# nihaomiao/CVPR23_LFDM

Measured on AMD Instinct MI355X. Metric: 40-frame 128x128 videos/sec (DDIM-100), higher is better.
Workload: dtype f32; 1 GPU; MUG 128x128, 40-frame DDIM-100 sample, batch=1 per GPU (BASELINE.json configs[1]); global_batch=1, frames=40, latent=32, image=128, sampler=DDIM-100 eta=1, cond_scale=1, parallelism=replicas x1 (videos sharded, no collective)

## Files before the change

cvpr23_lfdm_amd/csrc/attention.hip:

```cpp
#include <stdlib.h>
#include "attn_core.h"
#include "../../include/lfdm_hip.h"

namespace {

template <int LP>
__global__ __launch_bounds__(64) void attention_kernel(const float* __restrict__ qkv, float* __restrict__ out,
                                                       int frames, int hw, int mode, const float* __restrict__ bias,
                                                       const float* __restrict__ rot_cos,
                                                       const float* __restrict__ rot_sin) {
  constexpr int NT = LP / 16;

  const int lane = threadIdx.x & 63;
  const int l15 = lane & 15, lq = lane >> 4;
  const int L = mode == 0 ? frames : hw;
  const int64_t unit = blockIdx.x;
  const int64_t seq = unit / HEADS;
  const int head = (int)(unit - seq * HEADS);
  int64_t row0, tstride;
  if (mode == 0) {
    const int64_t b = seq / hw, pix = seq - b * hw;
    row0 = b * frames * hw + pix;
    tstride = hw;
  } else {
    row0 = seq * hw;
    tstride = 1;
  }
  const float* base = qkv + head * DH;

  float qf[NT][8], kf[NT][8];
#pragma unroll
  for (int ti = 0; ti < NT; ++ti) {
    const int t = ti * 16 + l15;
    float4 q0 = make_float4(0.f, 0.f, 0.f, 0.f), q1 = q0, k0 = q0, k1 = q0;
    if (t < L) {
      const float* src = base + (row0 + (int64_t)t * tstride) * QKV_LD + 8 * lq;
      q0 = *reinterpret_cast<const float4*>(src);
      q1 = *reinterpret_cast<const float4*>(src + 4);
      k0 = *reinterpret_cast<const float4*>(src + OUT_LD);
      k1 = *reinterpret_cast<const float4*>(src + OUT_LD + 4);
    }
    qf[ti][0] = q0.x * ATT_SCALE; qf[ti][1] = q0.y * ATT_SCALE; qf[ti][2] = q0.z * ATT_SCALE; qf[ti][3] = q0.w * ATT_SCALE;
    qf[ti][4] = q1.x * ATT_SCALE; qf[ti][5] = q1.y * ATT_SCALE; qf[ti][6] = q1.z * ATT_SCALE; qf[ti][7] = q1.w * ATT_SCALE;
    kf[ti][0] = k0.x; kf[ti][1] = k0.y; kf[ti][2] = k0.z; kf[ti][3] = k0.w;
    kf[ti][4] = k1.x; kf[ti][5] = k1.y; kf[ti][6] = k1.z; kf[ti][7] = k1.w;
  }
  float vf[2][4 * NT];
#pragma unroll
  for (int tj = 0; tj < NT; ++tj)
#pragma unroll
    for (int r = 0; r < 4; ++r) {
      const int t = 16 * tj + 4 * lq + r;
      vf[0][4 * tj + r] = vf[1][4 * tj + r] = 0.f;
      if (t < L) {
        const float* src = base + (row0 + (int64_t)t * tstride) * QKV_LD + 2 * OUT_LD;
        vf[0][4 * tj + r] = src[l15];
        vf[1][4 * tj + r] = src[16 + l15];
      }
    }
  if (rot_cos) {
#pragma unroll
    for (int ti = 0; ti < NT; ++ti) {
      const int t = ti * 16 + l15;
      if (t < L) {
#pragma unroll
        for (int pr = 0; pr < 4; ++pr) {
          const float c = rot_cos[t * 16 + 4 * lq + pr], sn = rot_sin[t * 16 + 4 * lq + pr];
          rot_pair(qf[ti][2 * pr], qf[ti][2 * pr + 1], c, sn);
          rot_pair(kf[ti][2 * pr], kf[ti][2 * pr + 1], c, sn);
        }
      }
    }
  }
  const bool bias_vec = bias && (L % 4 == 0) && ((((uintptr_t)bias) & 15) == 0);
  attend_store<NT, true>(qf, kf, vf, head, L, l15, lq, bias, bias_vec, out, row0, tstride);
}

__global__ __launch_bounds__(256) void linattn_context_kernel(const float* __restrict__ qkv, int hw,
                                                              float* __restrict__ ctx_out) {
  __shared__ float red[4][32];
  __shared__ float kmax[32];
  __shared__ float ek[64][33];
  __shared__ __attribute__((aligned(16))) float vv[64][36];
  const int tid = threadIdx.x;
  const int f = blockIdx.x >> 3, h = blockIdx.x & 7;
  const float* kbase = qkv + (int64_t)f * hw * QKV_LD + OUT_LD + h * DH;
  const float* vbase = kbase + OUT_LD;

  {
    const int c4 = tid & 7, part = tid >> 3;
    float4 m = make_float4(-3.0e38f, -3.0e38f, -3.0e38f, -3.0e38f);
    for (int n = part; n < hw; n += 128) {
      float4 v[4];
#pragma unroll
      for (int u = 0; u < 4; ++u) {
        const int nn = n + 32 * u;
        v[u] = nn < hw ? *reinterpret_cast<const float4*>(kbase + (int64_t)nn * QKV_LD + 4 * c4) : m;
      }
#pragma unroll
      for (int u = 0; u < 4; ++u) {
        m.x = fmaxf(m.x, v[u].x); m.y = fmaxf(m.y, v[u].y); m.z = fmaxf(m.z, v[u].z); m.w = fmaxf(m.w, v[u].w);
      }
    }
#pragma unroll
    for (int x = 8; x <= 32; x <<= 1) {
      m.x = fmaxf(m.x, __shfl_xor(m.x, x)); m.y = fmaxf(m.y, __shfl_xor(m.y, x));
      m.z = fmaxf(m.z, __shfl_xor(m.z, x)); m.w = fmaxf(m.w, __shfl_xor(m.w, x));
    }
    if ((tid & 63) < 8) {
      const int w = tid >> 6;
      red[w][4 * c4 + 0] = m.x; red[w][4 * c4 + 1] = m.y; red[w][4 * c4 + 2] = m.z; red[w][4 * c4 + 3] = m.w;
    }
    __syncthreads();
    if (tid < 32) kmax[tid] = fmaxf(fmaxf(red[0][tid], red[1][tid]), fmaxf(red[2][tid], red[3][tid]));
    __syncthreads();
  }

  const int d = tid >> 3, e0 = (tid & 7) * 4;
  float acc[4] = {0.f, 0.f, 0.f, 0.f};
  float ssum = 0.f;
  const int ln = tid >> 3, lc4 = tid & 7;
  float4 rk[2], rv[2];
  auto load_tile = [&](int n0) {
#pragma unroll
    for (int u = 0; u < 2; ++u) {
      const int n = n0 + ln + 32 * u;
      rk[u] = rv[u] = make_float4(0.f, 0.f, 0.f, 0.f);
      if (n < hw) {
// ... 53 lines not shown
  const int64_t row = (int64_t)f * hw + tok;
  const float* qp = qkv + row * QKV_LD + h * DH;
  float q[DH];
#pragma unroll
  for (int i = 0; i < DH / 4; ++i) {
    const float4 v = reinterpret_cast<const float4*>(qp)[i];
    q[4 * i] = v.x; q[4 * i + 1] = v.y; q[4 * i + 2] = v.z; q[4 * i + 3] = v.w;
  }
  float m = q[0];
#pragma unroll
  for (int i = 1; i < DH; ++i) m = fmaxf(m, q[i]);
  float sum = 0.f;
#pragma unroll
  for (int i = 0; i < DH; ++i) {
    q[i] = fast_exp(q[i] - m);
    sum += q[i];
  }
  const float scale = ATT_SCALE * fast_rcp(sum);
#pragma unroll
  for (int i = 0; i < DH; ++i) q[i] = q[i] * scale;
  float* op = out + row * OUT_LD + h * DH;
  const float* ch = cs + h * CS;
#pragma unroll
  for (int e4 = 0; e4 < DH / 4; ++e4) {
    float4 o = make_float4(0.f, 0.f, 0.f, 0.f);
#pragma unroll
    for (int dd = 0; dd < DH; ++dd) {
      const float4 c = *reinterpret_cast<const float4*>(ch + dd * DH + 4 * e4);
      o.x = fmaf(c.x, q[dd], o.x);
      o.y = fmaf(c.y, q[dd], o.y);
      o.z = fmaf(c.z, q[dd], o.z);
      o.w = fmaf(c.w, q[dd], o.w);
    }
    reinterpret_cast<float4*>(op)[e4] = o;
  }
}

}

extern "C" int lfdm_attention_cl_f32(const float* qkv, float* out, int batch, int frames, int hw,
                                     int mode, const float* bias, const float* rot_cos,
                                     const float* rot_sin, lfdm_stream_t stream_) {
  hipStream_t stream = (hipStream_t)stream_;
  const int L = mode == 0 ? frames : hw;
  if (!qkv || !out || batch <= 0 || frames <= 0 || hw <= 0 || (mode != 0 && mode != 1) ||
      L > 64 || ((rot_cos == nullptr) != (rot_sin == nullptr))) {
    lfdm_set_error("attention: unsupported shape (sequence length must be <= 64)");
    return LFDM_EINVAL;
  }
  const int64_t nseq = mode == 0 ? (int64_t)batch * hw : (int64_t)batch * frames;
  const int64_t units = nseq * HEADS;
  const dim3 grid((unsigned)units), block(64);
  lp_ladder(L, [&](auto lp) {
    LFDM_LAUNCH((attention_kernel<decltype(lp)::value>), grid, block, 0, stream, qkv, out, frames, hw, mode, bias, rot_cos, rot_sin);
  });
  return lfdm_check_launch("attention");
}

extern "C" size_t lfdm_linear_attention_ws_bytes(int n_frames) {
  return (size_t)n_frames * HEADS * DH * DH * sizeof(float);
}

extern "C" int lfdm_linear_attention_cl_f32(const float* qkv, float* out, int n_frames, int hw,
                                            void* ws, size_t ws_bytes, lfdm_stream_t stream_) {
  hipStream_t stream = (hipStream_t)stream_;
  if (!qkv || !out || n_frames <= 0 || hw <= 0) {
    lfdm_set_error("linear_attention: bad arguments");
    return LFDM_EINVAL;
  }
  if (!ws || ws_bytes < lfdm_linear_attention_ws_bytes(n_frames)) {
    lfdm_set_error("linear_attention: workspace too small");
    return LFDM_EWORKSPACE;
  }
  float* ctx = reinterpret_cast<float*>(ws);
  LFDM_LAUNCH(linattn_context_kernel, dim3(n_frames * HEADS), dim3(256), 0, stream, qkv, hw, ctx);
  LFDM_LAUNCH(linattn_output_kernel, dim3((hw + 31) / 32, n_frames), dim3(256), 0, stream, qkv,
              (const float*)ctx, hw, out);
  return lfdm_check_launch("linear_attention");
}
```

cvpr23_lfdm_amd/csrc/attention_fused.hip:

```cpp
#include <stdlib.h>

#include "attn_core.h"
#include "../../include/lfdm_hip.h"

namespace {

template <int LP, int C, bool ROT_RELOAD = false, bool WPACK = false>
__device__ __forceinline__ void tattn_heads(const float* __restrict__ x, int ldx, int head_begin, int heads_per_block,
                                            const float* __restrict__ wqkv, float* __restrict__ out, int frames, int hw, int64_t seq,
                                            const float* __restrict__ bias, const float* __restrict__ rot_cos,
                                            const float* __restrict__ rot_sin, float eps, float* o_lds) {
  constexpr int NT = LP / 16;
  constexpr int CQ = C / 4;

  const int lane = threadIdx.x & 63;
  const int l15 = lane & 15, lq = lane >> 4;
  const int L = frames;
  const int64_t b = seq / hw, pix = seq - b * hw;
  const int64_t row0 = b * frames * hw + pix;

  float xf[NT][CQ];
#pragma unroll
  for (int ti = 0; ti < NT; ++ti) {
    const int t = ti * 16 + l15;
    float s1 = 0.f, s2 = 0.f;
    if (t < L) {
      const float* src = x + (row0 + (int64_t)t * hw) * ldx + CQ * lq;
#pragma unroll
      for (int q = 0; q < CQ / 4; ++q) {
        const float4 v = *reinterpret_cast<const float4*>(src + 4 * q);
        xf[ti][4 * q] = v.x; xf[ti][4 * q + 1] = v.y; xf[ti][4 * q + 2] = v.z; xf[ti][4 * q + 3] = v.w;
        ln_accum(v, s1, s2);
      }
    } else {
#pragma unroll
      for (int s = 0; s < CQ; ++s) xf[ti][s] = 0.f;
    }
    float mean, rstd;
    ln_stats_slots4<false>(s1, s2, C, eps, mean, rstd);
    if (t < L) {
#pragma unroll
      for (int s = 0; s < CQ; ++s) xf[ti][s] = (xf[ti][s] - mean) * rstd;
    }
  }

  float rc[NT][4], rs[NT][4];
  if (rot_cos && !ROT_RELOAD) {
#pragma unroll
    for (int ti = 0; ti < NT; ++ti) {
      const int t = ti * 16 + l15;
      const int tt = t < L ? t : 0;
#pragma unroll
      for (int fi = 0; fi < 2; ++fi)
#pragma unroll
        for (int pr = 0; pr < 2; ++pr) {
          rc[ti][2 * fi + pr] = rot_cos[tt * 16 + 8 * fi + 2 * lq + pr];
          rs[ti][2 * fi + pr] = rot_sin[tt * 16 + 8 * fi + 2 * lq + pr];
        }
    }
  }
  const bool bias_vec = bias && (L % 4 == 0) && ((((uintptr_t)bias) & 15) == 0);

#pragma unroll 1
  for (int head = head_begin; head < head_begin + heads_per_block; ++head) {
    float qf[NT][8], kf[NT][8];
    {
      float wa[4][CQ];
#pragma unroll
      for (int g = 0; g < 4; ++g) {
        const float* wsrc = WPACK ? wqkv + ((int64_t)(((g >> 1) * HEADS + head) * 2 + (g & 1)) * (CQ / 4) * 64 + lane) * 4
                                  : wqkv + ((int64_t)((g >> 1) * OUT_LD + head * DH + 16 * (g & 1) + l15)) * C + CQ * lq;
#pragma unroll
        for (int q = 0; q < CQ / 4; ++q) {
          const float4 v = *reinterpret_cast<const float4*>(wsrc + (WPACK ? 256 * q : 4 * q));
          wa[g][4 * q] = v.x; wa[g][4 * q + 1] = v.y; wa[g][4 * q + 2] = v.z; wa[g][4 * q + 3] = v.w;
        }
      }
#pragma unroll
      for (int g = 0; g < 4; ++g) {
        f32x4 acc[NT];
#pragma unroll
        for (int ti = 0; ti < NT; ++ti) acc[ti] = (f32x4){0.f, 0.f, 0.f, 0.f};
#pragma unroll
        for (int s = 0; s < CQ; ++s)
#pragma unroll
          for (int ti = 0; ti < NT; ++ti) acc[ti] = mfma_16x16x4(wa[g][s], xf[ti][s], acc[ti]);
#pragma unroll
        for (int ti = 0; ti < NT; ++ti)
#pragma unroll
          for (int r = 0; r < 4; ++r) {
            if ((g >> 1) == 0) qf[ti][4 * (g & 1) + r] = acc[ti][r] * ATT_SCALE;
            else kf[ti][4 * (g & 1) + r] = acc[ti][r];
          }
      }
    }
    if (rot_cos) {
#pragma unroll
      for (int ti = 0; ti < NT; ++ti) {
#pragma unroll
        for (int fi = 0; fi < 2; ++fi)
#pragma unroll
          for (int pr = 0; pr < 2; ++pr) {
            float c, sn;
            if (ROT_RELOAD) {
              const int t = ti * 16 + l15, tt = t < L ? t : 0;
              c = rot_cos[tt * 16 + 8 * fi + 2 * lq + pr];
              sn = rot_sin[tt * 16 + 8 * fi + 2 * lq + pr];
            } else {
              c = rc[ti][2 * fi + pr];
              sn = rs[ti][2 * fi + pr];
            }
            rot_pair(qf[ti][4 * fi + 2 * pr], qf[ti][4 * fi + 2 * pr + 1], c, sn);
            rot_pair(kf[ti][4 * fi + 2 * pr], kf[ti][4 * fi + 2 * pr + 1], c, sn);
          }
      }
    }
    float vf[2][4 * NT];
    {
      float wb[2][CQ];
#pragma unroll
      for (int half = 0; half < 2; ++half) {
        const float* wsrc = WPACK ? wqkv + ((int64_t)((2 * HEADS + head) * 2 + half) * (CQ / 4) * 64 + lane) * 4
                                  : wqkv + ((int64_t)(2 * OUT_LD + head * DH + 16 * half + l15)) * C + CQ * lq;
#pragma unroll
        for (int q = 0; q < CQ / 4; ++q) {
          const float4 v = *reinterpret_cast<const float4*>(wsrc + (WPACK ? 256 * q : 4 * q));
          wb[half][4 * q] = v.x; wb[half][4 * q + 1] = v.y; wb[half][4 * q + 2] = v.z; wb[half][4 * q + 3] = v.w;
        }
      }
#pragma unroll
      for (int half = 0; half < 2; ++half) {
        f32x4 acc[NT];
#pragma unroll
        for (int ti = 0; ti < NT; ++ti) acc[ti] = (f32x4){0.f, 0.f, 0.f, 0.f};
#pragma unroll
        for (int s = 0; s < CQ; ++s)
#pragma unroll
          for (int ti = 0; ti < NT; ++ti) acc[ti] = mfma_16x16x4(xf[ti][s], wb[half][s], acc[ti]);
#pragma unroll
        for (int ti = 0; ti < NT; ++ti)
#pragma unroll
          for (int r = 0; r < 4; ++r) vf[half][4 * ti + r] = acc[ti][r];
      }
    }

    attend_store<NT, false>(qf, kf, vf, head, L, l15, lq, bias, bias_vec, out, row0, hw, o_lds);
  }
}

template <int LP, int C>
__global__ __launch_bounds__(64, 2) void temporal_attn_fused_kernel(const float* __restrict__ x, int ldx, int heads_per_block,
                                                                 const float* __restrict__ wqkv,
                                                                 float* __restrict__ out, int frames, int hw,
                                                                 const float* __restrict__ bias,
                                                                 const float* __restrict__ rot_cos,
                                                                 const float* __restrict__ rot_sin, float eps) {
  tattn_heads<LP, C>(x, ldx, blockIdx.y * heads_per_block, heads_per_block, wqkv, out, frames, hw, blockIdx.x, bias, rot_cos, rot_sin, eps, nullptr);
}

template <int LP, int LROWS, int NW>
__global__ __launch_bounds__(64 * NW, 2) void temporal_attn_fused_out_kernel(const float* __restrict__ x, int ldx,
                                                                          const float* __restrict__ wqkv, const float* __restrict__ wout,
                                                                          float* __restrict__ out, int ldo, int frames, int hw,
                                                                          const float* __restrict__ bias, const float* __restrict__ rot_cos,
                                                                          const float* __restrict__ rot_sin, float eps) {
  constexpr int C = 64, NT = LP / 16, CT = C / 16;
  __shared__ __attribute__((aligned(16))) float o_lds[LROWS * OUT_LD];
  const int wave = lfdm_uniform((int)(threadIdx.x >> 6));
  const int lane = threadIdx.x & 63, l15 = lane & 15, lq = lane >> 4;
  const int L = frames;
  const int64_t seq = blockIdx.x;
  tattn_heads<LP, C, (NW < 8), true>(x, ldx, wave * (HEADS / NW), HEADS / NW, wqkv, nullptr, frames, hw, seq, bias, rot_cos, rot_sin, eps, o_lds);
  __syncthreads();
  const int64_t b = seq / hw, pix = seq - b * hw;
  const int64_t row0 = b * frames * hw + pix;
  for (int tile = wave; tile < NT * CT; tile += NW) {
    const int ti = tile / CT, ct = tile - ti * CT;
    const int t = ti * 16 + l15;
    const int tr = t < L ? t : L - 1;
    const float* arow = o_lds + tr * OUT_LD;
    const float* brow = wout + ((int64_t)ct * (OUT_LD / 16) * 64 + lane) * 4;
    f32x4 acc = {0.f, 0.f, 0.f, 0.f}, acc1 = acc;
    float xr[4];
#pragma unroll
    for (int r = 0; r < 4; ++r) {
      const int tok = ti * 16 + 4 * lq + r;
      xr[r] = x[(row0 + (int64_t)(tok < L ? tok : L - 1) * hw) * ldx + ct * 16 + l15];
    }
#pragma unroll 4
    for (int S = 0; S < OUT_LD / 16; S += 2) {
      const float4 a = *reinterpret_cast<const float4*>(arow + (((4 * S + lq) ^ (tr & 15)) << 2));
      const float4 a1 = *reinterpret_cast<const float4*>(arow + (((4 * S + 4 + lq) ^ (tr & 15)) << 2));
      const float4 w = *reinterpret_cast<const float4*>(brow + 256 * S);
      const float4 w1 = *reinterpret_cast<const float4*>(brow + 256 * S + 256);
      acc = mfma_16x16x4(a.x, w.x, acc);
      acc1 = mfma_16x16x4(a1.x, w1.x, acc1);
      acc = mfma_16x16x4(a.y, w.y, acc);
      acc1 = mfma_16x16x4(a1.y, w1.y, acc1);
      acc = mfma_16x16x4(a.z, w.z, acc);
      acc1 = mfma_16x16x4(a1.z, w1.z, acc1);
      acc = mfma_16x16x4(a.w, w.w, acc);
      acc1 = mfma_16x16x4(a1.w, w1.w, acc1);
    }
#pragma unroll
    for (int r = 0; r < 4; ++r) acc[r] += acc1[r];
#pragma unroll
    for (int r = 0; r < 4; ++r) {
      const int tok = ti * 16 + 4 * lq + r;
      if (tok < L) {
        const int64_t row = row0 + (int64_t)tok * hw;
        out[row * ldo + ct * 16 + l15] = acc[r] + xr[r];
      }
    }
  }
}

template <int LP>
__global__ __launch_bounds__(64, 1) void temporal_attn_fused_wide_kernel(const float* __restrict__ x, int ldx, int channels,
                                                                      int heads_per_block, const float* __restrict__ wqkv,
                                                                      float* __restrict__ out, int frames, int hw,
                                                                      const float* __restrict__ bias,
                                                                      const float* __restrict__ rot_cos,
                                                                      const float* __restrict__ rot_sin, float eps) {
  constexpr int NT = LP / 16;
  const int lane = threadIdx.x & 63;
  const int l15 = lane & 15, lq = lane >> 4;
  const int L = frames;
  const int64_t seq = blockIdx.x;
  const int64_t b = seq / hw, pix = seq - b * hw;
  const int64_t row0 = b * frames * hw + pix;
  const int ncb = channels / 64;

  float mean[NT], rstd[NT];
#pragma unroll
  for (int ti = 0; ti < NT; ++ti) {
    const int t = ti * 16 + l15;
    float s1 = 0.f, s2 = 0.f;
    if (t < L) {
      const float* src = x + (row0 + (int64_t)t * hw) * ldx + 16 * lq;
      for (int cb = 0; cb < ncb; ++cb)
#pragma unroll
        for (int q = 0; q < 4; ++q) ln_accum(*reinterpret_cast<const float4*>(src + 64 * cb + 4 * q), s1, s2);
    }
    ln_stats_slots4<true>(s1, s2, channels, eps, mean[ti], rstd[ti]);
  }
  const bool bias_vec = bias && (L % 4 == 0) && ((((uintptr_t)bias) & 15) == 0);

  const int head_begin = blockIdx.y * heads_per_block;
#pragma unroll 1
  for (int head = head_begin; head < head_begin + heads_per_block; ++head) {
    f32x4 aq[2][NT], ak[2][NT], av[2][NT];
#pragma unroll
    for (int g = 0; g < 2; ++g)
#pragma unroll
      for (int ti = 0; ti < NT; ++ti) aq[g][ti] = ak[g][ti] = av[g][ti] = (f32x4){0.f, 0.f, 0.f, 0.f};
#pragma unroll 1
    for (int cb = 0; cb < ncb; ++cb) {
      float w[6][16];
#pragma unroll
      for (int g = 0; g < 6; ++g) {
        const float* wsrc = wqkv + ((int64_t)((g >> 1) * OUT_LD + head * DH + 16 * (g & 1) + l15)) * channels + 64 * cb + 16 * lq;
#pragma unroll
        for (int q = 0; q < 4; ++q) {
          const float4 v = *reinterpret_cast<const float4*>(wsrc + 4 * q);
          w[g][4 * q] = v.x; w[g][4 * q + 1] = v.y; w[g][4 * q + 2] = v.z; w[g][4 * q + 3] = v.w;
        }
      }
#pragma unroll
      for (int ti = 0; ti < NT; ++ti) {
        const int t = ti * 16 + l15;
        float xf[16];
        if (t < L) {
          const float* src = x + (row0 + (int64_t)t * hw) * ldx + 64 * cb + 16 * lq;
#pragma unroll
          for (int q = 0; q < 4; ++q) {
            const float4 v = *reinterpret_cast<const float4*>(src + 4 * q);
            xf[4 * q] = (v.x - mean[ti]) * rstd[ti]; xf[4 * q + 1] = (v.y - mean[ti]) * rstd[ti];
            xf[4 * q + 2] = (v.z - mean[ti]) * rstd[ti]; xf[4 * q + 3] = (v.w - mean[ti]) * rstd[ti];
          }
        } else {
#pragma unroll
          for (int s2 = 0; s2 < 16; ++s2) xf[s2] = 0.f;
        }
#pragma unroll
        for (int s2 = 0; s2 < 16; ++s2) {
          aq[0][ti] = mfma_16x16x4(w[0][s2], xf[s2], aq[0][ti]);
          aq[1][ti] = mfma_16x16x4(w[1][s2], xf[s2], aq[1][ti]);
          ak[0][ti] = mfma_16x16x4(w[2][s2], xf[s2], ak[0][ti]);
          ak[1][ti] = mfma_16x16x4(w[3][s2], xf[s2], ak[1][ti]);
          av[0][ti] = mfma_16x16x4(xf[s2], w[4][s2], av[0][ti]);
          av[1][ti] = mfma_16x16x4(xf[s2], w[5][s2], av[1][ti]);
        }
      }
    }
    float qf[NT][8], kf[NT][8], vf[2][4 * NT];
#pragma unroll
    for (int ti = 0; ti < NT; ++ti)
#pragma unroll
      for (int fi = 0; fi < 2; ++fi)
#pragma unroll
        for (int r = 0; r < 4; ++r) {
          qf[ti][4 * fi + r] = aq[fi][ti][r] * ATT_SCALE;
          kf[ti][4 * fi + r] = ak[fi][ti][r];
          vf[fi][4 * ti + r] = av[fi][ti][r];
        }
    if (rot_cos) {
#pragma unroll
      for (int ti = 0; ti < NT; ++ti) {
        const int t = ti * 16 + l15;
        const int tt = t < L ? t : 0;
#pragma unroll
        for (int fi = 0; fi < 2; ++fi)
#pragma unroll
          for (int pr = 0; pr < 2; ++pr) {
            const float c = rot_cos[tt * 16 + 8 * fi + 2 * lq + pr], sn = rot_sin[tt * 16 + 8 * fi + 2 * lq + pr];
            rot_pair(qf[ti][4 * fi + 2 * pr], qf[ti][4 * fi + 2 * pr + 1], c, sn);
            rot_pair(kf[ti][4 * fi + 2 * pr], kf[ti][4 * fi + 2 * pr + 1], c, sn);
          }
      }
    }
    attend_store<NT, false>(qf, kf, vf, head, L, l15, lq, bias, bias_vec, out, row0, hw);
  }
}

int launch_fused_wide(const float* x, int ldx, int channels, const float* wqkv, float* out, int batch, int frames, int hw,
                      const float* bias, const float* rot_cos, const float* rot_sin, float eps, hipStream_t stream) {
  const int64_t nseq = (int64_t)batch * hw;
  int hpb = 8;
  while (hpb > 1 && nseq * (HEADS / hpb) < 2048) hpb >>= 1;
  const dim3 grid((unsigned)nseq, (unsigned)(HEADS / hpb)), block(64);
  lp_ladder(frames, [&](auto lp) {
    LFDM_LAUNCH((temporal_attn_fused_wide_kernel<decltype(lp)::value>), grid, block, 0, stream, x, ldx, channels, hpb, wqkv, out, frames, hw, bias, rot_cos, rot_sin, eps);
  });
  return lfdm_check_launch("temporal_attention_fused_wide");
}

template <int C>
int launch_fused(const float* x, int ldx, const float* wqkv, float* out, int batch, int frames, int hw, const float* bias,
                 const float* rot_cos, const float* rot_sin, float eps, hipStream_t stream) {
  const int64_t nseq = (int64_t)batch * hw;
  int hpb = 8;
  while (hpb > 1 && nseq * (HEADS / hpb) < 2048) hpb >>= 1;
  if (const char* e = lfdm_knob("LFDM_TATTN_HPB")) {
    const int v = atoi(e);
    if (v == 1 || v == 2 || v == 4 || v == 8) hpb = v;
  }
  const dim3 grid((unsigned)nseq, (unsigned)(HEADS / hpb)), block(64);
  lp_ladder(frames, [&](auto lp) {
    LFDM_LAUNCH((temporal_attn_fused_kernel<decltype(lp)::value, C>), grid, block, 0, stream, x, ldx, hpb, wqkv, out, frames, hw, bias, rot_cos, rot_sin, eps);
  });
  return lfdm_check_launch("temporal_attention_fused");
}

template <int LP, int LROWS>
int launch_fused_out_lp(const float* x, int ldx, const float* wqkv, const float* wout, float* out, int ldo, int batch, int frames, int hw,
                        const float* bias, const float* rot_cos, const float* rot_sin, float eps, hipStream_t stream) {
  const int64_t nseq = (int64_t)batch * hw;
  int nw = 2;
  while (nw < 8 && nseq * nw < 2048) nw <<= 1;
  if (const char* e = getenv("LFDM_TATTN_OUT_NW")) {
    const int v = atoi(e);
    if (v == 1 || v == 2 || v == 4 || v == 8) nw = v;
  }
  const dim3 grid((unsigned)nseq);
  lfdm_ladder<1, 2, 4, 8>(nw, [&](auto nwc) {
    constexpr int NW = decltype(nwc)::value;
    LFDM_LAUNCH((temporal_attn_fused_out_kernel<LP, LROWS, NW>), grid, dim3(64 * NW), 0, stream, x, ldx, wqkv, wout, out, ldo, frames, hw, bias, rot_cos, rot_sin, eps);
  });
  return lfdm_check_launch("temporal_attention_fused_out");
}

}

extern "C" int lfdm_temporal_attention_fused_out_cl_f32(const float* x, int ldx, int channels, const float* wqkv, const float* wout,
                                                        float* out, int ldo, int batch, int frames, int hw, const float* bias,
                                                        const float* rot_cos, const float* rot_sin, float ln_eps, lfdm_stream_t stream_) {
  hipStream_t stream = (hipStream_t)stream_;
  if (!x || !wqkv || !wout || !out || batch <= 0 || frames <= 0 || frames > 64 || hw <= 0 || channels != 64 || ldx < 64 || ldx % 4 != 0 ||
      ldo < 64 || (((uintptr_t)x | (uintptr_t)wqkv | (uintptr_t)wout) & 15) || ((rot_cos == nullptr) != (rot_sin == nullptr)) || out == x) {
    lfdm_set_error("temporal_attention_fused_out: needs C == 64, frames <= 64, 16-byte aligned rows, out != x");
    return LFDM_EINVAL;
  }
  return lp_ladder(frames, [&](auto lp) {
    constexpr int LP = decltype(lp)::value;
    if (LP == 48 && frames <= 40)
      return launch_fused_out_lp<48, 40>(x, ldx, wqkv, wout, out, ldo, batch, frames, hw, bias, rot_cos, rot_sin, ln_eps, stream);
    return launch_fused_out_lp<LP, LP>(x, ldx, wqkv, wout, out, ldo, batch, frames, hw, bias, rot_cos, rot_sin, ln_eps, stream);
  });
}

extern "C" int lfdm_temporal_attention_fused_cl_f32(const float* x, int ldx, int channels, const float* wqkv, float* out,
                                                    int batch, int frames, int hw, const float* bias,
                                                    const float* rot_cos, const float* rot_sin, float ln_eps,
                                                    lfdm_stream_t stream_) {
  hipStream_t stream = (hipStream_t)stream_;
  if (!x || !wqkv || !out || batch <= 0 || frames <= 0 || frames > 64 || hw <= 0 || ldx < channels || ldx % 4 != 0 ||
      (((uintptr_t)x | (uintptr_t)wqkv) & 15) || ((rot_cos == nullptr) != (rot_sin == nullptr)) ||
      channels < 64 || channels % 64 != 0) {
    lfdm_set_error("temporal_attention_fused: needs C % 64 == 0, frames <= 64, 16-byte aligned rows");
    return LFDM_EINVAL;
  }
  if (channels == 64) return launch_fused<64>(x, ldx, wqkv, out, batch, frames, hw, bias, rot_cos, rot_sin, ln_eps, stream);
  return launch_fused_wide(x, ldx, channels, wqkv, out, batch, frames, hw, bias, rot_cos, rot_sin, ln_eps, stream);
}
```

cvpr23_lfdm_amd/csrc/attn_core.h:

```cpp
#pragma once
#include "lfdm_device.h"

constexpr int HEADS = 8;
constexpr int DH = 32;
constexpr int QKV_LD = 3 * HEADS * DH;
constexpr int OUT_LD = HEADS * DH;
constexpr float ATT_SCALE = 0.17677669529663687f;

__device__ __forceinline__ void seq_rows(int64_t seq, int mode, int frames, int hw, int64_t& row0, int64_t& tstride) {
  if (mode == 0) {
    const int64_t b = seq / hw, pix = seq - b * hw;
    row0 = b * frames * hw + pix;
    tstride = hw;
  } else {
    row0 = seq * hw;
    tstride = 1;
  }
}

__device__ __forceinline__ void rot_pair(float& x, float& y, float c, float sn) {
  const float x0 = x, y0 = y;
  x = x0 * c - y0 * sn;
  y = y0 * c + x0 * sn;
}

template <int NT, bool FAST_RCP>
__device__ __forceinline__ float softmax_tile(f32x4 (&st)[NT], int head, int L, int qt, int lq, const float* __restrict__ bias, bool bias_vec) {
  float m = -3.0e38f;
#pragma unroll
  for (int tj = 0; tj < NT; ++tj) {
    float bv[4] = {0.f, 0.f, 0.f, 0.f};
    const int key0 = tj * 16 + lq * 4;
    if (bias && qt < L && key0 < L) {
      const float* bp = bias + ((int64_t)head * L + qt) * L + key0;
      if (bias_vec) {
        const float4 b4 = *reinterpret_cast<const float4*>(bp);
        bv[0] = b4.x; bv[1] = b4.y; bv[2] = b4.z; bv[3] = b4.w;
      } else {
#pragma unroll
        for (int r = 0; r < 4; ++r) bv[r] = (key0 + r < L) ? bp[r] : 0.f;
      }
    }
#pragma unroll
    for (int r = 0; r < 4; ++r) {
      const float v = (key0 + r >= L) ? -3.0e38f : st[tj][r] + bv[r];
      st[tj][r] = v;
      m = fmaxf(m, v);
    }
  }
  m = fmaxf(m, __shfl_xor(m, 16));
  m = fmaxf(m, __shfl_xor(m, 32));
  float sum = 0.f;
#pragma unroll
  for (int tj = 0; tj < NT; ++tj)
#pragma unroll
    for (int r = 0; r < 4; ++r) {
      const float e = (tj * 16 + lq * 4 + r) < L ? fast_exp(st[tj][r] - m) : 0.f;
      st[tj][r] = e;
      sum += e;
    }
  sum += __shfl_xor(sum, 16);
  sum += __shfl_xor(sum, 32);
  return FAST_RCP ? fast_rcp(sum) : 1.0f / sum;
}

template <int NT, bool FAST_RCP>
__device__ __forceinline__ void attend_store(const float (&qf)[NT][8], const float (&kf)[NT][8], const float (&vf)[2][4 * NT],
                                             int head, int L, int l15, int lq, const float* __restrict__ bias, bool bias_vec,
                                             float* __restrict__ out, int64_t row0, int64_t tstride, float* o_lds = nullptr) {
  f32x4 st[NT][NT];
#pragma unroll
  for (int ti = 0; ti < NT; ++ti)
#pragma unroll
    for (int tj = 0; tj < NT; ++tj) {
      f32x4 acc = {0.f, 0.f, 0.f, 0.f};
#pragma unroll
      for (int s = 0; s < 8; ++s) acc = mfma_16x16x4(kf[tj][s], qf[ti][s], acc);
      st[ti][tj] = acc;
    }
#pragma unroll
  for (int ti = 0; ti < NT; ++ti) {
    const float inv = softmax_tile<NT, FAST_RCP>(st[ti], head, L, ti * 16 + l15, lq, bias, bias_vec);
#pragma unroll
    for (int tj = 0; tj < NT; ++tj)
#pragma unroll
      for (int r = 0; r < 4; ++r) st[ti][tj][r] = st[ti][tj][r] * inv;
  }

#pragma unroll
  for (int ti = 0; ti < NT; ++ti) {
    f32x4 o[2];
    o[0] = (f32x4){0.f, 0.f, 0.f, 0.f};
    o[1] = o[0];
#pragma unroll
    for (int tj = 0; tj < NT; ++tj)
#pragma unroll
      for (int r = 0; r < 4; ++r) {
        o[0] = mfma_16x16x4(st[ti][tj][r], vf[0][4 * tj + r], o[0]);
        o[1] = mfma_16x16x4(st[ti][tj][r], vf[1][4 * tj + r], o[1]);
      }
#pragma unroll
    for (int r = 0; r < 4; ++r) {
      const int t = ti * 16 + lq * 4 + r;
      if (t < L) {
        if (o_lds) {
#pragma unroll
          for (int half = 0; half < 2; ++half) {
            const int c = head * DH + 16 * half + l15;
            o_lds[t * OUT_LD + ((((c >> 2) ^ (t & 15)) << 2) | (c & 3))] = o[half][r];
          }
        } else {
          float* dst = out + (row0 + t * tstride) * OUT_LD + head * DH;
          dst[l15] = o[0][r];
          dst[16 + l15] = o[1][r];
        }
      }
    }
  }
}

__device__ __forceinline__ void ln_accum(const float4& v, float& s1, float& s2) {
  s1 += (v.x + v.y) + (v.z + v.w);
  s2 += (v.x * v.x + v.y * v.y) + (v.z * v.z + v.w * v.w);
}
template <bool DIVIDE>
__device__ __forceinline__ void ln_stats_slots4(float s1, float s2, int channels, float eps, float& mean, float& rstd) {
  s1 += __shfl_xor(s1, 16); s2 += __shfl_xor(s2, 16);
  s1 += __shfl_xor(s1, 32); s2 += __shfl_xor(s2, 32);
  mean = DIVIDE ? s1 / (float)channels : s1 * (1.0f / (float)channels);
  float var = (DIVIDE ? s2 / (float)channels : s2 * (1.0f / (float)channels)) - mean * mean;
  if (var < 0.f) var = 0.f;
  rstd = 1.0f / sqrtf(var + eps);
}

template <class F>
inline auto lp_ladder(int L, F&& f) { return lfdm_ladder<16, 32, 48, 64>(L, f); }
```

cvpr23_lfdm_amd/csrc/lfdm_device.h:

```cpp
#pragma once
#include <stddef.h>
#include <stdint.h>
#include <type_traits>

#if defined(LFDM_EMU_BUILD)
#include "hip_emu.h"
typedef emu_f32x16 f32x16;
typedef emu_f32x4 f32x4;
#define LFDM_LAUNCH(kern, grid, block, smem, stream, ...) \
  emu::launch(grid, block, smem, [=]() { kern(__VA_ARGS__); })
static inline f32x16 mfma_32x32x2(float a, float b, f32x16 c) { return emu_mfma_32x32x2(a, b, c); }
static inline f32x4 mfma_16x16x4(float a, float b, f32x4 c) { return emu_mfma_16x16x4(a, b, c); }
static inline f32x4 mfma_4x4x1(float a, float b, f32x4 c) { return emu_mfma_4x4x1(a, b, c); }
struct lfdm_bf16x8 { uint16_t h[8]; };
static inline uint16_t lfdm_f32_to_bf16(float f) {
  uint32_t u;
  memcpy(&u, &f, 4);
  if ((u & 0x7fffffffu) > 0x7f800000u) return (uint16_t)((u >> 16) | 0x40u);
  u += 0x7fffu + ((u >> 16) & 1u);
  return (uint16_t)(u >> 16);
}
static inline float lfdm_bf16_to_f32(uint16_t h) {
  const uint32_t u = (uint32_t)h << 16;
  float f;
// ... 152 lines not shown
__device__ __forceinline__ void lfdm_gload_f4(f32x4& dst, const float* p) {
  asm volatile("global_load_dwordx4 %0, %1, off offset:%2" : "=v"(dst) : "v"(p), "n"(OFF) : "memory");
}
template <int N> __device__ __forceinline__ void lfdm_vmwait() { asm volatile("s_waitcnt vmcnt(%0)" ::"n"(N) : "memory"); }
template <int N> __device__ __forceinline__ void lfdm_vmwait(f32x4& a) { asm volatile("s_waitcnt vmcnt(%1)" : "+v"(a) : "n"(N) : "memory"); }
template <int N> __device__ __forceinline__ void lfdm_vmwait(f32x4& a, f32x4& b) {
  asm volatile("s_waitcnt vmcnt(%2)" : "+v"(a), "+v"(b) : "n"(N) : "memory");
}
template <int N> __device__ __forceinline__ void lfdm_vmwait(f32x4& a, f32x4& b, f32x4& c, f32x4& d) {
  asm volatile("s_waitcnt vmcnt(%4)" : "+v"(a), "+v"(b), "+v"(c), "+v"(d) : "n"(N) : "memory");
}
__device__ __forceinline__ void lfdm_tie(f32x4& a) { asm volatile("" : "+v"(a)::"memory"); }
__device__ __forceinline__ int lfdm_uniform(int v) { return __builtin_amdgcn_readfirstlane(v); }
#endif

#if defined(LFDM_EMU_BUILD)
#define LFDM_DRAIN_STORES() ((void)0)
#define LFDM_FENCE_RELEASE_AGENT() ((void)0)
#define LFDM_FENCE_ACQUIRE_AGENT() ((void)0)
static inline unsigned lfdm_ticket_take(unsigned* c) { return __atomic_fetch_add(c, 1u, __ATOMIC_SEQ_CST); }
static inline void lfdm_ticket_reset(unsigned* c) { __atomic_store_n(c, 0u, __ATOMIC_SEQ_CST); }
#else
#define LFDM_DRAIN_STORES() asm volatile("s_waitcnt vmcnt(0)" ::: "memory")
#define LFDM_FENCE_RELEASE_AGENT() __builtin_amdgcn_fence(__ATOMIC_RELEASE, "agent")
#define LFDM_FENCE_ACQUIRE_AGENT() __builtin_amdgcn_fence(__ATOMIC_ACQUIRE, "agent")
__device__ __forceinline__ unsigned lfdm_ticket_take(unsigned* c) {
  return __hip_atomic_fetch_add(c, 1u, __ATOMIC_RELAXED, __HIP_MEMORY_SCOPE_AGENT);
}
__device__ __forceinline__ void lfdm_ticket_reset(unsigned* c) {
  __hip_atomic_store(c, 0u, __ATOMIC_RELAXED, __HIP_MEMORY_SCOPE_AGENT);
}
#endif

#if defined(__HIP_DEVICE_COMPILE__) && !defined(__gfx950__) && !defined(LFDM_EMU_BUILD)
#error "fence-free hand-off (lfdm_agent_store_u64 / lfdm_agent_load_u64 / lfdm_ticket_take) validated on gfx950 only: re-validate, or use LFDM_FENCE_RELEASE_AGENT / LFDM_FENCE_ACQUIRE_AGENT, before building for another target"
#endif
#if defined(LFDM_EMU_BUILD)
static inline void lfdm_agent_store_u64(unsigned long long* p, unsigned long long v) { __atomic_store_n(p, v, __ATOMIC_SEQ_CST); }
static inline unsigned long long lfdm_agent_load_u64(const unsigned long long* p) { return __atomic_load_n(p, __ATOMIC_SEQ_CST); }
static inline unsigned lfdm_agent_load_u32(const unsigned* p) { return __atomic_load_n(p, __ATOMIC_SEQ_CST); }
static inline void lfdm_sleep() {}
#else
__device__ __forceinline__ void lfdm_agent_store_u64(unsigned long long* p, unsigned long long v) {
  __hip_atomic_store(p, v, __ATOMIC_RELAXED, __HIP_MEMORY_SCOPE_AGENT);
}
__device__ __forceinline__ unsigned long long lfdm_agent_load_u64(const unsigned long long* p) {
  return __hip_atomic_load(p, __ATOMIC_RELAXED, __HIP_MEMORY_SCOPE_AGENT);
}
__device__ __forceinline__ unsigned lfdm_agent_load_u32(const unsigned* p) { return __hip_atomic_load(p, __ATOMIC_RELAXED, __HIP_MEMORY_SCOPE_AGENT); }
__device__ __forceinline__ void lfdm_sleep() { __builtin_amdgcn_s_sleep(2); }
#endif

#if defined(LFDM_EMU_BUILD)
static inline void lfdm_wave_lds_sync() { emu::wave_sync(); }
#else
__device__ __forceinline__ void lfdm_wave_lds_sync() {
  __builtin_amdgcn_fence(__ATOMIC_RELEASE, "wavefront");
  __builtin_amdgcn_wave_barrier();
  __builtin_amdgcn_fence(__ATOMIC_ACQUIRE, "wavefront");
}
#endif

__device__ __forceinline__ float wave_sum(float v) {
#pragma unroll
  for (int m = 32; m >= 1; m >>= 1) v += __shfl_xor(v, m);
  return v;
}
__device__ __forceinline__ float wave_max(float v) {
#pragma unroll
  for (int m = 32; m >= 1; m >>= 1) v = fmaxf(v, __shfl_xor(v, m));
  return v;
}
#if defined(LFDM_EMU_BUILD)
static inline float fast_exp(float x) { return expf(x); }
static inline float fast_rcp(float x) { return 1.0f / x; }
#else
__device__ __forceinline__ float fast_exp(float x) { return __expf(x); }
__device__ __forceinline__ float fast_rcp(float x) { return __builtin_amdgcn_rcpf(x); }
#endif
__device__ __forceinline__ float sigmoidf_(float x) { return 1.0f / (1.0f + expf(-x)); }
__device__ __forceinline__ float siluf_(float x) { return x / (1.0f + expf(-x)); }

#if defined(LFDM_EMU_BUILD)
static inline float silu_fast_(float x) { return x / (1.0f + expf(-x)); }
#else
__device__ __forceinline__ float silu_fast_(float x) { return x * __builtin_amdgcn_rcpf(1.0f + __expf(-x)); }
#endif

#if defined(LFDM_TUNING_KNOBS) || defined(LFDM_EMU_BUILD)
static inline const char* lfdm_knob(const char* name) { return getenv(name); }
#else
static inline const char* lfdm_knob(const char*) { return nullptr; }
#endif

__device__ __forceinline__ float apply_act(float v, int act) {
  if (act == 1) return v > 0.f ? v : 0.f;
  if (act == 2) return sigmoidf_(v);
  if (act == 3) return siluf_(v);
  return v;
}

extern "C" void lfdm_set_error(const char* msg);
int lfdm_check_launch(const char* what);
```

Baseline: 4.125 videos/s.

## Software-pipeline attention score MFMA with softmax VALU per query tile

```diff
diff --git a/cvpr23_lfdm_amd/csrc/attention.hip b/cvpr23_lfdm_amd/csrc/attention.hip
--- a/cvpr23_lfdm_amd/csrc/attention.hip
+++ b/cvpr23_lfdm_amd/csrc/attention.hip
@@ -4,7 +4,7 @@
 
 namespace {
 
-template <int LP>
+template <int LP, bool PIPE>
 __global__ __launch_bounds__(64) void attention_kernel(const float* __restrict__ qkv, float* __restrict__ out,
                                                        int frames, int hw, int mode, const float* __restrict__ bias,
                                                        const float* __restrict__ rot_cos,
@@ -73,7 +73,7 @@
     }
   }
   const bool bias_vec = bias && (L % 4 == 0) && ((((uintptr_t)bias) & 15) == 0);
-  attend_store<NT, true>(qf, kf, vf, head, L, l15, lq, bias, bias_vec, out, row0, tstride);
+  attend_store<NT, true, PIPE>(qf, kf, vf, head, L, l15, lq, bias, bias_vec, out, row0, tstride);
 }
 
 __global__ __launch_bounds__(256) void linattn_context_kernel(const float* __restrict__ qkv, int hw,
@@ -233,7 +233,12 @@
   const int64_t units = nseq * HEADS;
   const dim3 grid((unsigned)units), block(64);
   lp_ladder(L, [&](auto lp) {
-    LFDM_LAUNCH((attention_kernel<decltype(lp)::value>), grid, block, 0, stream, qkv, out, frames, hw, mode, bias, rot_cos, rot_sin);
+    constexpr int LP = decltype(lp)::value;
+    constexpr bool CAN_PIPE = LP != 32;
+    if (CAN_PIPE && bias_by_quads(bias, L))
+      LFDM_LAUNCH((attention_kernel<LP, CAN_PIPE>), grid, block, 0, stream, qkv, out, frames, hw, mode, bias, rot_cos, rot_sin);
+    else
+      LFDM_LAUNCH((attention_kernel<LP, false>), grid, block, 0, stream, qkv, out, frames, hw, mode, bias, rot_cos, rot_sin);
   });
   return lfdm_check_launch("attention");
 }
diff --git a/cvpr23_lfdm_amd/csrc/attention_fused.hip b/cvpr23_lfdm_amd/csrc/attention_fused.hip
--- a/cvpr23_lfdm_amd/csrc/attention_fused.hip
+++ b/cvpr23_lfdm_amd/csrc/attention_fused.hip
@@ -5,11 +5,34 @@
 
 namespace {
 
-template <int LP, int C, bool ROT_RELOAD = false, bool WPACK = false>
+#ifdef LFDM_TATTN_STAMP
+struct CycleProbe {
+  long long t, acc[8];
+  __device__ __forceinline__ void start() {
+    for (int i = 0; i < 8; ++i) acc[i] = 0;
+    t = clock64();
+  }
+  __device__ __forceinline__ void lap(int i) {
+    LFDM_SCHED_FENCE();
+    const long long now = clock64();
+    acc[i] += now - t;
+    t = now;
+    LFDM_SCHED_FENCE();
+  }
+};
+long long* tattn_stamps = nullptr;
+#define TATTN_STAMP_PARAM , long long* stamps
+#define TATTN_STAMP_ARG , tattn_stamps
+#else
+#define TATTN_STAMP_PARAM
+#define TATTN_STAMP_ARG
+#endif
+
+template <int LP, int C, bool ROT_RELOAD = false, bool WPACK = false, bool PIPE = false, bool TO_LDS = false, class PROBE = NoProbe>
 __device__ __forceinline__ void tattn_heads(const float* __restrict__ x, int ldx, int head_begin, int heads_per_block,
                                             const float* __restrict__ wqkv, float* __restrict__ out, int frames, int hw, int64_t seq,
                                             const float* __restrict__ bias, const float* __restrict__ rot_cos,
-                                            const float* __restrict__ rot_sin, float eps, float* o_lds) {
+                                            const float* __restrict__ rot_sin, float eps, PROBE&& probe = NoProbe{}) {
   constexpr int NT = LP / 16;
   constexpr int CQ = C / 4;
 
@@ -60,6 +83,7 @@
     }
   }
   const bool bias_vec = bias && (L % 4 == 0) && ((((uintptr_t)bias) & 15) == 0);
+  probe.lap(4);
 
 #pragma unroll 1
   for (int head = head_begin; head < head_begin + heads_per_block; ++head) {
@@ -144,34 +168,42 @@
       }
     }
 
-    attend_store<NT, false>(qf, kf, vf, head, L, l15, lq, bias, bias_vec, out, row0, hw, o_lds);
-  }
-}
-
-template <int LP, int C>
+    probe.lap(0);
+    attend_store<NT, false, PIPE, TO_LDS>(qf, kf, vf, head, L, l15, lq, bias, bias_vec, out, row0, hw, probe);
+  }
+}
+
+template <int LP, int C, bool PIPE>
 __global__ __launch_bounds__(64, 2) void temporal_attn_fused_kernel(const float* __restrict__ x, int ldx, int heads_per_block,
                                                                  const float* __restrict__ wqkv,
                                                                  float* __restrict__ out, int frames, int hw,
                                                                  const float* __restrict__ bias,
                                                                  const float* __restrict__ rot_cos,
                                                                  const float* __restrict__ rot_sin, float eps) {
-  tattn_heads<LP, C>(x, ldx, blockIdx.y * heads_per_block, heads_per_block, wqkv, out, frames, hw, blockIdx.x, bias, rot_cos, rot_sin, eps, nullptr);
-}
-
-template <int LP, int LROWS, int NW>
+  tattn_heads<LP, C, false, false, PIPE>(x, ldx, blockIdx.y * heads_per_block, heads_per_block, wqkv, out, frames, hw, blockIdx.x, bias, rot_cos, rot_sin, eps);
+}
+
+template <int LP, int LROWS, int NW, bool PIPE>
 __global__ __launch_bounds__(64 * NW, 2) void temporal_attn_fused_out_kernel(const float* __restrict__ x, int ldx,
                                                                           const float* __restrict__ wqkv, const float* __restrict__ wout,
                                                                           float* __restrict__ out, int ldo, int frames, int hw,
                                                                           const float* __restrict__ bias, const float* __restrict__ rot_cos,
-                                                                          const float* __restrict__ rot_sin, float eps) {
+                                                                          const float* __restrict__ rot_sin, float eps TATTN_STAMP_PARAM) {
   constexpr int C = 64, NT = LP / 16, CT = C / 16;
   __shared__ __attribute__((aligned(16))) float o_lds[LROWS * OUT_LD];
   const int wave = lfdm_uniform((int)(threadIdx.x >> 6));
   const int lane = threadIdx.x & 63, l15 = lane & 15, lq = lane >> 4;
   const int L = frames;
   const int64_t seq = blockIdx.x;
-  tattn_heads<LP, C, (NW < 8), true>(x, ldx, wave * (HEADS / NW), HEADS / NW, wqkv, nullptr, frames, hw, seq, bias, rot_cos, rot_sin, eps, o_lds);
+#ifdef LFDM_TATTN_STAMP
+  CycleProbe probe;
+  probe.start();
+#else
+  NoProbe probe;
+#endif
+  tattn_heads<LP, C, (NW < 8), true, PIPE, true>(x, ldx, wave * (HEADS / NW), HEADS / NW, wqkv, o_lds, frames, hw, seq, bias, rot_cos, rot_sin, eps, probe);
   __syncthreads();
+  probe.lap(5);
   const int64_t b = seq / hw, pix = seq - b * hw;
   const int64_t row0 = b * frames * hw + pix;
   for (int tile = wave; tile < NT * CT; tile += NW) {
@@ -213,9 +245,14 @@
       }
     }
   }
-}
-
-template <int LP>
+#ifdef LFDM_TATTN_STAMP
+  probe.lap(6);
+  if (stamps && lane == 0 && blockIdx.x < 256)
+    for (int i = 0; i < 8; ++i) stamps[((int64_t)blockIdx.x * 8 + wave) * 8 + i] = probe.acc[i];
+#endif
+}
+
+template <int LP, bool PIPE>
 __global__ __launch_bounds__(64, 1) void temporal_attn_fused_wide_kernel(const float* __restrict__ x, int ldx, int channels,
                                                                       int heads_per_block, const float* __restrict__ wqkv,
                                                                       float* __restrict__ out, int frames, int hw,
@@ -319,7 +356,7 @@
           }
       }
     }
-    attend_store<NT, false>(qf, kf, vf, head, L, l15, lq, bias, bias_vec, out, row0, hw);
+    attend_store<NT, false, PIPE>(qf, kf, vf, head, L, l15, lq, bias, bias_vec, out, row0, hw);
   }
 }
 
@@ -330,7 +367,11 @@
   while (hpb > 1 && nseq * (HEADS / hpb) < 2048) hpb >>= 1;
   const dim3 grid((unsigned)nseq, (unsigned)(HEADS / hpb)), block(64);
   lp_ladder(frames, [&](auto lp) {
-    LFDM_LAUNCH((temporal_attn_fused_wide_kernel<decltype(lp)::value>), grid, block, 0, stream, x, ldx, channels, hpb, wqkv, out, frames, hw, bias, rot_cos, rot_sin, eps);
+    constexpr int LP = decltype(lp)::value;
+    if (bias_by_quads(bias, frames))
+      LFDM_LAUNCH((temporal_attn_fused_wide_kernel<LP, true>), grid, block, 0, stream, x, ldx, channels, hpb, wqkv, out, frames, hw, bias, rot_cos, rot_sin, eps);
+    else
+      LFDM_LAUNCH((temporal_attn_fused_wide_kernel<LP, false>), grid, block, 0, stream, x, ldx, channels, hpb, wqkv, out, frames, hw, bias, rot_cos, rot_sin, eps);
   });
   return lfdm_check_launch("temporal_attention_fused_wide");
 }
@@ -347,7 +388,12 @@
   }
   const dim3 grid((unsigned)nseq, (unsigned)(HEADS / hpb)), block(64);
   lp_ladder(frames, [&](auto lp) {
-    LFDM_LAUNCH((temporal_attn_fused_kernel<decltype(lp)::value, C>), grid, block, 0, stream, x, ldx, hpb, wqkv, out, frames, hw, bias, rot_cos, rot_sin, eps);
+    constexpr int LP = decltype(lp)::value;
+    constexpr bool CAN_PIPE = LP <= 32;
+    if (CAN_PIPE && bias_by_quads(bias, frames))
+      LFDM_LAUNCH((temporal_attn_fused_kernel<LP, C, CAN_PIPE>), grid, block, 0, stream, x, ldx, hpb, wqkv, out, frames, hw, bias, rot_cos, rot_sin, eps);
+    else
+      LFDM_LAUNCH((temporal_attn_fused_kernel<LP, C, false>), grid, block, 0, stream, x, ldx, hpb, wqkv, out, frames, hw, bias, rot_cos, rot_sin, eps);
   });
   return lfdm_check_launch("temporal_attention_fused");
 }
@@ -365,12 +411,24 @@
   const dim3 grid((unsigned)nseq);
   lfdm_ladder<1, 2, 4, 8>(nw, [&](auto nwc) {
     constexpr int NW = decltype(nwc)::value;
-    LFDM_LAUNCH((temporal_attn_fused_out_kernel<LP, LROWS, NW>), grid, dim3(64 * NW), 0, stream, x, ldx, wqkv, wout, out, ldo, frames, hw, bias, rot_cos, rot_sin, eps);
+#if defined(LFDM_TATTN_STAMP) && LFDM_TATTN_STAMP == 2
+    constexpr bool CAN_PIPE = false;
+#else
+    constexpr bool CAN_PIPE = !(LP == 64 && NW == 4);
+#endif
+    if (CAN_PIPE && bias_by_quads(bias, frames))
+      LFDM_LAUNCH((temporal_attn_fused_out_kernel<LP, LROWS, NW, CAN_PIPE>), grid, dim3(64 * NW), 0, stream, x, ldx, wqkv, wout, out, ldo, frames, hw, bias, rot_cos, rot_sin, eps TATTN_STAMP_ARG);
+    else
+      LFDM_LAUNCH((temporal_attn_fused_out_kernel<LP, LROWS, NW, false>), grid, dim3(64 * NW), 0, stream, x, ldx, wqkv, wout, out, ldo, frames, hw, bias, rot_cos, rot_sin, eps TATTN_STAMP_ARG);
   });
   return lfdm_check_launch("temporal_attention_fused_out");
 }
 
 }
+
+#ifdef LFDM_TATTN_STAMP
+extern "C" void lfdm_tattn_stamp_buffer(void* p) { tattn_stamps = (long long*)p; }
+#endif
 
 extern "C" int lfdm_temporal_attention_fused_out_cl_f32(const float* x, int ldx, int channels, const float* wqkv, const float* wout,
                                                         float* out, int ldo, int batch, int frames, int hw, const float* bias,
diff --git a/cvpr23_lfdm_amd/csrc/attn_core.h b/cvpr23_lfdm_amd/csrc/attn_core.h
--- a/cvpr23_lfdm_amd/csrc/attn_core.h
+++ b/cvpr23_lfdm_amd/csrc/attn_core.h
@@ -24,14 +24,18 @@
   y = y0 * c + x0 * sn;
 }
 
-template <int NT, bool FAST_RCP>
-__device__ __forceinline__ float softmax_tile(f32x4 (&st)[NT], int head, int L, int qt, int lq, const float* __restrict__ bias, bool bias_vec) {
-  float m = -3.0e38f;
+template <int NT, bool GUARDED>
+__device__ __forceinline__ void bias_quads(f32x4 (&bq)[NT], int head, int L, int qt, int lq, const float* __restrict__ bias, bool bias_vec,
+                                           bool clamp_q = true) {
 #pragma unroll
   for (int tj = 0; tj < NT; ++tj) {
-    float bv[4] = {0.f, 0.f, 0.f, 0.f};
+    f32x4 bv = {0.f, 0.f, 0.f, 0.f};
     const int key0 = tj * 16 + lq * 4;
-    if (bias && qt < L && key0 < L) {
+    if (!GUARDED) {
+      const float* brow = bias + ((int64_t)head * L + (clamp_q && qt > L - 1 ? L - 1 : qt)) * L;
+      const float4 b4 = *reinterpret_cast<const float4*>(brow + (tj == NT - 1 && key0 > L - 4 ? L - 4 : key0));
+      bv[0] = b4.x; bv[1] = b4.y; bv[2] = b4.z; bv[3] = b4.w;
+    } else if (bias && qt < L && key0 < L) {
       const float* bp = bias + ((int64_t)head * L + qt) * L + key0;
       if (bias_vec) {
         const float4 b4 = *reinterpret_cast<const float4*>(bp);
@@ -41,9 +45,19 @@
         for (int r = 0; r < 4; ++r) bv[r] = (key0 + r < L) ? bp[r] : 0.f;
       }
     }
-#pragma unroll
-    for (int r = 0; r < 4; ++r) {
-      const float v = (key0 + r >= L) ? -3.0e38f : st[tj][r] + bv[r];
+    bq[tj] = bv;
+  }
+}
+
+template <int NT, bool FAST_RCP>
+__device__ __forceinline__ float softmax_tile(f32x4 (&st)[NT], const f32x4 (&bq)[NT], int L, int lq) {
+  float m = -3.0e38f;
+#pragma unroll
+  for (int tj = 0; tj < NT; ++tj) {
+    const int key0 = tj * 16 + lq * 4;
+#pragma unroll
+    for (int r = 0; r < 4; ++r) {
+      const float v = (key0 + r >= L) ? -3.0e38f : st[tj][r] + bq[tj][r];
       st[tj][r] = v;
       m = fmaxf(m, v);
     }
@@ -63,21 +77,105 @@
   sum += __shfl_xor(sum, 32);
   return FAST_RCP ? fast_rcp(sum) : 1.0f / sum;
 }
-
 template <int NT, bool FAST_RCP>
+__device__ __forceinline__ float softmax_tile(f32x4 (&st)[NT], int head, int L, int qt, int lq, const float* __restrict__ bias, bool bias_vec) {
+  f32x4 bq[NT];
+  bias_quads<NT, true>(bq, head, L, qt, lq, bias, bias_vec);
+  return softmax_tile<NT, FAST_RCP>(st, bq, L, lq);
+}
+
+template <int NT>
+__device__ __forceinline__ void score_tile(f32x4 (&st)[NT], const float (&q)[8], const float (&kf)[NT][8]) {
+#pragma unroll
+  for (int tj = 0; tj < NT; ++tj) {
+    f32x4 acc = {0.f, 0.f, 0.f, 0.f};
+#pragma unroll
+    for (int s = 0; s < 8; ++s) acc = mfma_16x16x4(kf[tj][s], q[s], acc);
+    st[tj] = acc;
+  }
+}
+
+template <int NT>
+__device__ __forceinline__ void pv_tile(f32x4 (&o)[2], const f32x4 (&p)[NT], const float (&vf)[2][4 * NT]) {
+  o[0] = (f32x4){0.f, 0.f, 0.f, 0.f};
+  o[1] = o[0];
+#pragma unroll
+  for (int tj = 0; tj < NT; ++tj)
+#pragma unroll
+    for (int r = 0; r < 4; ++r) {
+      o[0] = mfma_16x16x4(p[tj][r], vf[0][4 * tj + r], o[0]);
+      o[1] = mfma_16x16x4(p[tj][r], vf[1][4 * tj + r], o[1]);
+    }
+}
+
+template <bool TO_LDS>
+__device__ __forceinline__ void store_token(const f32x4 (&o)[2], int r, int t, int head, int l15, float* __restrict__ out, int64_t row0,
+                                            int64_t tstride) {
+  if (TO_LDS) {
+#pragma unroll
+    for (int half = 0; half < 2; ++half) {
+      const int c = head * DH + 16 * half + l15;
+      out[t * OUT_LD + ((((c >> 2) ^ (t & 15)) << 2) | (c & 3))] = o[half][r];
+    }
+  } else {
+    float* dst = out + (row0 + t * tstride) * OUT_LD + head * DH;
+    dst[l15] = o[0][r];
+    dst[16 + l15] = o[1][r];
+  }
+}
+
+struct NoProbe {
+  __device__ __forceinline__ void lap(int) {}
+};
+
+template <int NT, bool FAST_RCP, bool TO_LDS, class PROBE>
+__device__ __forceinline__ void attend_tiles(const float (&qf)[NT][8], const float (&kf)[NT][8], const float (&vf)[2][4 * NT],
+                                             int head, int L, int l15, int lq, const float* __restrict__ bias,
+                                             float* __restrict__ out, int64_t row0, int64_t tstride, PROBE& probe) {
+  f32x4 st[2][NT], bq[NT];
+  bias_quads<NT, false>(bq, head, L, l15, lq, bias, true, NT == 1);
+  score_tile<NT>(st[0], qf[0], kf);
+  LFDM_SCHED_FENCE();
+  probe.lap(1);
+#pragma unroll
+  for (int ti = 0; ti < NT; ++ti) {
+    f32x4 (&p)[NT] = st[ti & 1];
+    if (ti + 1 < NT) score_tile<NT>(st[(ti + 1) & 1], qf[ti + 1], kf);
+    const float inv = softmax_tile<NT, FAST_RCP>(p, bq, L, lq);
+#pragma unroll
+    for (int tj = 0; tj < NT; ++tj)
+#pragma unroll
+      for (int r = 0; r < 4; ++r) p[tj][r] = p[tj][r] * inv;
+    if (ti + 1 < NT) {
+#pragma unroll
+      for (int i = 0; i < 8 * NT; ++i) {
+        LFDM_SCHED_GROUP(LFDM_SG_MFMA, 1);
+        LFDM_SCHED_GROUP(LFDM_SG_VALU, 4);
+      }
+    }
+    probe.lap(2);
+    if (ti + 1 < NT) bias_quads<NT, false>(bq, head, L, (ti + 1) * 16 + l15, lq, bias, true, ti + 1 == NT - 1);
+    f32x4 o[2];
+    pv_tile<NT>(o, p, vf);
+#pragma unroll
+    for (int r = 0; r < 4; ++r) {
+      const int t = ti * 16 + lq * 4 + r;
+      if (ti < NT - 1 || t < L) store_token<TO_LDS>(o, r, t, head, l15, out, row0, tstride);
+    }
+    LFDM_SCHED_FENCE();
+    probe.lap(3);
+  }
+}
+
+template <int NT, bool FAST_RCP, bool PIPE = false, bool TO_LDS = false, class PROBE = NoProbe>
 __device__ __forceinline__ void attend_store(const float (&qf)[NT][8], const float (&kf)[NT][8], const float (&vf)[2][4 * NT],
                                              int head, int L, int l15, int lq, const float* __restrict__ bias, bool bias_vec,
-                                             float* __restrict__ out, int64_t row0, int64_t tstride, float* o_lds = nullptr) {
+                                             float* __restrict__ out, int64_t row0, int64_t tstride, PROBE&& probe = NoProbe{}) {
+  if (PIPE) return attend_tiles<NT, FAST_RCP, TO_LDS>(qf, kf, vf, head, L, l15, lq, bias, out, row0, tstride, probe);
   f32x4 st[NT][NT];
 #pragma unroll
-  for (int ti = 0; ti < NT; ++ti)
-#pragma unroll
-    for (int tj = 0; tj < NT; ++tj) {
-      f32x4 acc = {0.f, 0.f, 0.f, 0.f};
-#pragma unroll
-      for (int s = 0; s < 8; ++s) acc = mfma_16x16x4(kf[tj][s], qf[ti][s], acc);
-      st[ti][tj] = acc;
-    }
+  for (int ti = 0; ti < NT; ++ti) score_tile<NT>(st[ti], qf[ti], kf);
+  probe.lap(1);
 #pragma unroll
   for (int ti = 0; ti < NT; ++ti) {
     const float inv = softmax_tile<NT, FAST_RCP>(st[ti], head, L, ti * 16 + l15, lq, bias, bias_vec);
@@ -86,37 +184,18 @@
 #pragma unroll
       for (int r = 0; r < 4; ++r) st[ti][tj][r] = st[ti][tj][r] * inv;
   }
-
+  probe.lap(2);
 #pragma unroll
   for (int ti = 0; ti < NT; ++ti) {
     f32x4 o[2];
-    o[0] = (f32x4){0.f, 0.f, 0.f, 0.f};
-    o[1] = o[0];
-#pragma unroll
-    for (int tj = 0; tj < NT; ++tj)
-#pragma unroll
-      for (int r = 0; r < 4; ++r) {
-        o[0] = mfma_16x16x4(st[ti][tj][r], vf[0][4 * tj + r], o[0]);
-        o[1] = mfma_16x16x4(st[ti][tj][r], vf[1][4 * tj + r], o[1]);
-      }
+    pv_tile<NT>(o, st[ti], vf);
 #pragma unroll
     for (int r = 0; r < 4; ++r) {
       const int t = ti * 16 + lq * 4 + r;
-      if (t < L) {
-        if (o_lds) {
-#pragma unroll
-          for (int half = 0; half < 2; ++half) {
-            const int c = head * DH + 16 * half + l15;
-            o_lds[t * OUT_LD + ((((c >> 2) ^ (t & 15)) << 2) | (c & 3))] = o[half][r];
-          }
-        } else {
-          float* dst = out + (row0 + t * tstride) * OUT_LD + head * DH;
-          dst[l15] = o[0][r];
-          dst[16 + l15] = o[1][r];
-        }
-      }
-    }
-  }
+      if (t < L) store_token<TO_LDS>(o, r, t, head, l15, out, row0, tstride);
+    }
+  }
+  probe.lap(3);
 }
 
 __device__ __forceinline__ void ln_accum(const float4& v, float& s1, float& s2) {
@@ -133,5 +212,7 @@
   rstd = 1.0f / sqrtf(var + eps);
 }
 
+inline bool bias_by_quads(const float* bias, int L) { return bias && L % 4 == 0 && (((uintptr_t)bias) & 15) == 0; }
+
 template <class F>
 inline auto lp_ladder(int L, F&& f) { return lfdm_ladder<16, 32, 48, 64>(L, f); }
diff --git a/cvpr23_lfdm_amd/csrc/lfdm_device.h b/cvpr23_lfdm_amd/csrc/lfdm_device.h
--- a/cvpr23_lfdm_amd/csrc/lfdm_device.h
+++ b/cvpr23_lfdm_amd/csrc/lfdm_device.h
@@ -228,6 +228,16 @@
 #endif
 
 #if defined(LFDM_EMU_BUILD)
+#define LFDM_SCHED_FENCE() ((void)0)
+#define LFDM_SCHED_GROUP(mask, n) ((void)0)
+#else
+#define LFDM_SCHED_FENCE() __builtin_amdgcn_sched_barrier(0)
+#define LFDM_SCHED_GROUP(mask, n) __builtin_amdgcn_sched_group_barrier(mask, n, 0)
+#endif
+#define LFDM_SG_VALU 0x002
+#define LFDM_SG_MFMA 0x008
+
+#if defined(LFDM_EMU_BUILD)
 static inline void lfdm_wave_lds_sync() { emu::wave_sync(); }
 #else
 __device__ __forceinline__ void lfdm_wave_lds_sync() {
```

Measured after the change: 4.170 videos/s (median of 6 runs). 1.01x the previous value.
